# pvjosue/CWFA

Hardware: AMD Instinct MI355X
Metric: volumes/sec inverse-pass @512×512×96 fp32; NLL match vs ref (1/2/4/8 GPU) (higher is better)
Workload: dtype f32 (storage, accumulation, wavelets, couplings); convolution products on the bf16 matrix cores from an exact three-way bf16 split of both fp32 operands, six products per fp32 product: fp32-equivalent; plain-fp32-MFMA figure: fp32_mfma; 1 GPU; 512x512x96 volume, 4-scale CWFA (CAT blocks, 64 ch) + LRNN inverse, z=0, batch 1/GPU, random-init weights (BASELINE.json configs[2]); precision=split, parallelism=replicated x1 (independent volumes per GPU, no collective)

## Files before the change

cwfa_amd/_lib.py:

```python
import ctypes as C
import os

_HERE = os.path.dirname(os.path.abspath(__file__))
LIB_PATH = os.path.join(_HERE, "libcwfa_hip.so")

CLAMP = {"NONE": 0, "ATAN": 1, "TANH": 2, "SIGMOID": 3}
ACT = {None: 0, "none": 0, "elu": 1, "prelu": 2, "gelu": 3, "relu": 4}
CHAIN_MAX = 8

c_f32p = C.c_void_p
c_i64p = C.c_void_p
c_f64p = C.c_void_p


class AffineStage(C.Structure):
    _fields_ = [("s_raw", c_f32p), ("t", c_f32p), ("s_bs", C.c_int64), ("t_bs", C.c_int64), ("clamp_kind", C.c_int),
                ("clamp", C.c_float), ("pre_scale", C.c_float), ("t_neg_div_sqrt2", C.c_int), ("perm", c_i64p),
                ("perm_axis", C.c_int), ("gin", C.c_int)]


class Chain(C.Structure):
    _fields_ = [("n_stages", C.c_int), ("stage", AffineStage * CHAIN_MAX), ("src_c", C.c_void_p), ("src_h", C.c_void_p)]


# ... 45 lines not shown
    "cwfa_layernorm_apply_f32": (i, [p, p, p, p, f, p, i, i64, p]),
    "cwfa_attention_combine_f32": (i, [p, p, p, p, p, p, p, p, i, i, i64, p]),
    "cwfa_scale_channels_f32": (i, [p, p, p, i, i, i64, p]),
    "cwfa_axpby_f32": (i, [p, p, f, f, p, i64, p]),
    "cwfa_bn_running_update_f32": (i, [p, C.c_double, f, p, p, p, i, p]),
    "cwfa_bn_finish_f32": (i, [p, d, p, p, p, f, i, p, p, f, p, p, f, f, i, p, p, i, i, p]),
    "cwfa_chain_bwd_f32": (i, [p, p, C.POINTER(Chain), C.POINTER(ChainGrads), p, p, i, i, i, i, i64, i64, i64, f, f, i, p, p]),
    "cwfa_affine_bwd_f32": (i, [p, p, C.POINTER(AffineStage), i, i, i, i, i, i64, i64, p, p, p, p, p]),
    "cwfa_chain_inv_bwd_f32": (i, [p, p, C.POINTER(Chain), C.POINTER(ChainGrads), i, i, i, i, i64, i64, f, i, i, p, p, p, p]),
    "cwfa_conv2d_wgrad_workspace_bytes": (i64, [i, i, i, i, i, i]),
    "cwfa_conv2d_wgrad_f32": (i, [p, p, p, p, p, i, i, i, i, i, i, i64, i64, f, p]),
    "cwfa_elu_bwd_f32": (i, [p, p, p, p, i, i64, i64, i64, i64, i64, p]),
    "cwfa_conv3d_hidden_fwd_f32": (i, [p, p, p, p, i, i, i, i, i, p]),
    "cwfa_conv3d_hidden_bwd_f32": (i, [p, p, p, p, p, p, i, i, i, i, i, p]),
    "cwfa_conv3d_input_bwd_f32": (i, [p, p, p, i, i, i, i, i, p]),
    "cwfa_conv3d_wgrad_workspace_bytes": (i64, [i, i, i, i]),
    "cwfa_conv3d_wgrad_f32": (i, [p, p, p, p, p, i, i, i, i, i, i, i, f, p]),
    "cwfa_prelu_bwd_f32": (i, [p, p, p, p, p, i, i64, i64, i64, i64, p]),
    "cwfa_plane_affine_f32": (i, [p, p, p, i, p, p, i, i, i64, i64, i64, i64, p]),
    "cwfa_bn_bwd_stats_f32": (i, [p, p, p, p, i, i, i64, i64, i64, p]),
    "cwfa_bn_act_bwd_f32": (i, [p, p, p, i, p, p, p, p, p, i, i, i64, i64, i64, i64, p]),
    "cwfa_maxpool2_bwd_f32": (i, [p, p, p, p, i, i, i, i, p]),
    "cwfa_gelu_f32": (i, [p, p, p, i64, i, p]),
    "cwfa_layernorm_bwd_f32": (i, [p, p, p, p, p, p, p, p, p, i, i64, p]),
    "cwfa_attention_bwd_f32": (i, [p, p, p, p, p, p, p, p, p, i, i, i64, p]),
    "cwfa_split_workspace_bytes": (i64, [i, i, i64]),
    "cwfa_split_input_f32": (i, [p, p, i, i, i64, i64, p, p, i64, p, i64, p]),
    "cwfa_conv_split_packed_bytes": (i64, [i, i, i]),
    "cwfa_conv_split_pack_f32": (i, [p, p, i, i, i, i, p]),
    "cwfa_conv_split_f32": (i, [p, p, p, i, i, i, i, i, i, i64, C.POINTER(ConvOpts), p]),
    "cwfa_conv3x3_split_packed_bytes": (i64, [i, i]),
    "cwfa_conv3x3_split_pack_f32": (i, [p, p, i, i, p]),
    "cwfa_conv3x3_split_f32": (i, [p, p, p, i, i, i, i, i, i64, i64, C.POINTER(ConvOpts), p]),
    "cwfa_conv7x7_split_packed_bytes": (i64, [i, i]),
    "cwfa_conv7x7_split_pack_f32": (i, [p, p, i, i, p]),
    "cwfa_conv7x7_split_f32": (i, [p, p, p, i, i, i, i, i, i64, i64, C.POINTER(ConvOpts), p]),
    "cwfa_couple_rows": (i, [i, p]),
    "cwfa_conv3x3_split_couple_f32": (i, [p, p, p, i, i, i, i, i64, C.POINTER(Couple), p]),
    "cwfa_subnet_layer_split_packed_bytes": (i64, []),
    "cwfa_subnet_layer_split_pack_f32": (i, [p, p, p, p]),
    "cwfa_subnet_layer_split_f32": (i, [p, p, p, p, p, i, i, i, i64, i64, i, p]),
    "cwfa_subnet_layer_split_tape_f32": (i, [p, p, p, p, p, p, i, i, i, i64, i64, i64, p]),
    "cwfa_subnet_layer_first_packed_bytes": (i64, []),
    "cwfa_subnet_layer_first_pack_f32": (i, [p, p, p, i, p, p]),
    "cwfa_subnet_layer_first_f32": (i, [p, p, p, p, p, p, i, i, i, i, i64, i64, i64, i, p]),
    "cwfa_extract_views_f32": (i, [p, p, p, i, i, i, i, i, i, f, f, i64, p]),
}
del i, i64, f, d, p

_lib = None


class CwfaHipError(RuntimeError):
    pass


def lib():
    global _lib
    if _lib is None:
        if not os.path.exists(LIB_PATH):
            raise CwfaHipError(
                f"{LIB_PATH} not found: build the HIP extension first (python -m cwfa_amd.build, or "
                f"__graft_entry__.build()).  cwfa_amd has no CPU / PyTorch fallback.")
        import torch
        h = C.CDLL(LIB_PATH)
        for name, (res, args) in SIGNATURES.items():
# ... 14 lines not shown
```

cwfa_amd/csrc/conv_split3x3.hip:

```cpp
#include "conv_internal.h"

extern int g_cwfa_split_products;
extern int g_cwfa_split_xcd_map;
extern int g_cwfa_split_rows16;
extern int g_cwfa_split_operand;

namespace {

constexpr int TR = 8, TC = 32;

template <int KS, int RPW = 4>
struct XG {
    static constexpr int TRW = 2 * RPW, NT = 2 * RPW;
    static constexpr int PAD = KS / 2, XR = TRW + 2 * PAD, XC = TC + 2 * PAD, NTAP = KS * KS;
    static constexpr int EPK = XR * XC;
    static constexpr int KHB = KS == 7 ? 8512 : RPW == 8 ? 9792 : 5440;
    static constexpr int XPB = 2 * KHB;
    static constexpr int XB = 3 * XPB;
    static constexpr bool SPECIAL = KS == 3 && RPW == 4;
    static constexpr int NEK = SPECIAL ? 2 : 3;
    static_assert(EPK * 16 <= KHB && KHB % 256 == 64 && 2 * EPK <= 512 * NEK, "staging entry map");
    static_assert(!SPECIAL || (EPK > 256 && EPK <= 384), "3x3 staging entry map");
    static_assert(KS == 3 || RPW == 4, "7x7: 8-row tiles");
};
// ... 446 lines not shown
                                                            int nchunks, int nsteps, int64_t total, int ntap) {
    const int64_t i = (int64_t)blockIdx.x * blockDim.x + threadIdx.x;
    if (i >= total) return;
    const int col = (int)(i % CT), g = (int)((i / CT) % 4), s = (int)((i / (4 * CT)) % nsteps), ctile = (int)(i / ((int64_t)4 * CT * nsteps));
    const int u = 2 * s + (g >> 1), chunk = u / ntap, tap = u % ntap, co = ctile * CT + col;
    unsigned short pc[3][8];
#pragma unroll
    for (int j = 0; j < 8; ++j) {
        const int ci = chunk * 16 + (g & 1) * 8 + j;
        float v = 0.f;
        if (co < Cout && ci < Cin && chunk < nchunks) v = w[((int64_t)co * Cin + ci) * ntap + tap];
        __bf16 a1, a2, a3;
        if constexpr (F16) {
            cwfa_split3<false, true>(v, a1, a2, a3);
            a2 = a3 = __builtin_bit_cast(__bf16, (unsigned short)0);
        } else {
            cwfa_split3<true>(v, a1, a2, a3);
        }
        pc[0][j] = __builtin_bit_cast(unsigned short, a1);
        pc[1][j] = __builtin_bit_cast(unsigned short, a2);
        pc[2][j] = __builtin_bit_cast(unsigned short, a3);
    }
#pragma unroll
    for (int q = 0; q < 3; ++q) {
        uint4 v4;
        v4.x = pc[q][0] | ((unsigned)pc[q][1] << 16);
        v4.y = pc[q][2] | ((unsigned)pc[q][3] << 16);
        v4.z = pc[q][4] | ((unsigned)pc[q][5] << 16);
        v4.w = pc[q][6] | ((unsigned)pc[q][7] << 16);
        out[(((int64_t)ctile * nsteps + s) * 3 + q) * 4 * CT + g * CT + col] = v4;
    }
}

inline int mpw_of(int Cout) { return Cout > 128 ? 4 : Cout > 96 ? 2 : Cout > 64 ? 3 : Cout > 48 ? 1 : Cout > 32 ? 3 : Cout > 16 ? 2 : 1; }
inline int wm_of(int Cout) { return Cout > 96 ? 4 : Cout > 64 ? 2 : Cout > 48 ? 4 : 1; }
inline int ct_of(int Cout) { return 16 * mpw_of(Cout) * wm_of(Cout); }
inline int nsteps_of(int Cin, int ntap = 9) { return ntap * (((Cin + 15) / 16 + 1) / 2); }

template <int MPW, bool SIX, bool ADD, int ACT1, int KS = 3, int RPW = 4, int WM = 4, bool F16 = false>
int launch(const SParams& p, hipStream_t stream) {
    typedef Geo<MPW, KS, RPW, WM> G;
    constexpr int TRW = XG<KS, RPW>::TRW;
    auto kern = &conv3x3_split_kernel<MPW, SIX, ADD, ACT1, KS, RPW, WM, F16>;
    static bool attr_set = false;
    if (!attr_set) {
        hipError_t e = hipFuncSetAttribute(reinterpret_cast<const void*>(kern), hipFuncAttributeMaxDynamicSharedMemorySize, G::LDS);
        if (e != hipSuccess) {
            cwfa_set_error("cwfa_conv3x3_split_f32: hipFuncSetAttribute(%d bytes LDS): %s", G::LDS, hipGetErrorString(e));
            return CWFA_E_HIP;
        }
        attr_set = true;
    }
    const int tiles_y = (p.H + TRW - 1) / TRW, ctiles = (p.Cout + G::CT - 1) / G::CT;
    SParams q = p;
    q.ntiles = p.tiles_x * tiles_y;
    q.ctiles = ctiles;
    q.xcd_map = g_cwfa_split_xcd_map;
    if ((int64_t)q.ntiles * ctiles >= (1ll << 31)) {
        cwfa_set_error("cwfa_conv3x3_split_f32: grid too large");
        return CWFA_E_SHAPE;
    }
    hipLaunchKernelGGL(kern, dim3((unsigned)(q.ntiles * ctiles), 1, p.B), dim3(512), G::LDS, stream, q);
    CWFA_LAUNCH_CHECK("cwfa_conv3x3_split_f32");
    return CWFA_OK;
}

inline int split_op() { return g_cwfa_split_products != 1 ? 0 : g_cwfa_split_operand ? 2 : 1; }

template <int MPW, bool ADD, int ACT1, int KS = 3, int RPW = 4, int WM = 4>
int launch_op(int op, const SParams& p, hipStream_t st) {
    if (op == 0) return launch<MPW, true, ADD, ACT1, KS, RPW, WM>(p, st);
    if (op == 1) return launch<MPW, false, ADD, ACT1, KS, RPW, WM>(p, st);
    return launch<MPW, false, ADD, ACT1, KS, RPW, WM, true>(p, st);
}

template <int MPW>
int launch_epi(int op, const SParams& p, hipStream_t st) {
    const bool plain = !p.o.residual && p.o.act2 == CWFA_ACT_NONE;
    if (p.o.in_add) {
        if (plain && p.o.act == CWFA_ACT_PRELU) return launch_op<MPW, true, CWFA_ACT_PRELU>(op, p, st);
        return launch_op<MPW, true, EPI_RUNTIME>(op, p, st);
    }
    if (plain && p.o.act == CWFA_ACT_PRELU) return launch_op<MPW, false, CWFA_ACT_PRELU>(op, p, st);
    if (plain && p.o.act == CWFA_ACT_NONE) return launch_op<MPW, false, CWFA_ACT_NONE>(op, p, st);
    return launch_op<MPW, false, EPI_RUNTIME>(op, p, st);
}

}

static int couple_row_source(int n, int r) {
    int j, which;
    if (n <= 32) {
        const int wm = r >> 4, g = (r >> 2) & 3, q = r & 3;
        j = 8 * wm + 2 * g + (q & 1);
        which = q >> 1;
    } else {
        const int wm = r >> 5;
        which = (r >> 4) & 1;
        j = 16 * wm + (r & 15);
    }
    return j < n ? which * n + j : -1;
}

extern "C" int cwfa_couple_rows(int n, int* rows) {
    if (n <= 0 || n > 64) return -1;
    const int total = n <= 32 ? 64 : 128;
// ... 104 lines not shown
    CWFA_REQUIRE((int64_t)(Cin + 64) * H * W * 4 < (1ll << 31) && (int64_t)(Cout + 64 * mpw) * H * W * 4 < (1ll << 31) &&
                     (int64_t)(p.nsteps + 2) * 3 * 4 * 64 * mpw * 16 < (1ll << 31), CWFA_E_SHAPE,
                 "cwfa_conv3x3_split_f32: one sample's input / output / one cout tile's weights must stay below 2 GiB");
    CWFA_REQUIRE((int64_t)p.tiles_x * ((H + TR - 1) / TR) < (1ll << 31) && B <= 65535, CWFA_E_SHAPE, "cwfa_conv3x3_split_f32: grid too large");
    hipStream_t st = (hipStream_t)stream;
    const int op = split_op();
    const int wm = wm_of(Cout);
    if (wm != 4) {
        CWFA_REQUIRE(!p.o.in_scale && !p.o.in_add && !p.o.out_blocked8, CWFA_E_INVAL,
                     "cwfa_conv3x3_split_f32: banks with <= 48 or 65 .. 96 outputs take no load-side prologue and write NCHW");
        const bool plain = !p.o.residual && p.o.act2 == CWFA_ACT_NONE;
        const int epi = plain && p.o.act == CWFA_ACT_NONE ? 0 : plain && p.o.act == CWFA_ACT_PRELU ? 1 : 2;
#define CWFA_NARROW(M, W_)                                                                                                                   \
    do {                                                                                                                                     \
        if (epi == 0) return launch_op<M, false, CWFA_ACT_NONE, 3, 8, W_>(op, p, st);                                                    \
        if (epi == 1) return launch_op<M, false, CWFA_ACT_PRELU, 3, 8, W_>(op, p, st);                                                   \
        return launch_op<M, false, EPI_RUNTIME, 3, 8, W_>(op, p, st);                                                                    \
    } while (0)
        if (mpw == 3 && wm == 2) CWFA_NARROW(3, 2);
        if (mpw == 3) CWFA_NARROW(3, 1);
        if (mpw == 2) CWFA_NARROW(2, 1);
        CWFA_NARROW(1, 1);
#undef CWFA_NARROW
    }
    if (mpw == 4) return launch_epi<4>(op, p, st);
    if (mpw == 2) return launch_epi<2>(op, p, st);
    if (g_cwfa_split_rows16 && H > 8 && !p.o.in_scale && !p.o.in_add && !p.o.residual && p.o.act == CWFA_ACT_NONE && p.o.act2 == CWFA_ACT_NONE)
        return launch_op<2, false, CWFA_ACT_NONE, 3, 8, 2>(op, p, st);
    if (g_cwfa_split_rows16 && H > 8 && !p.o.in_scale && !p.o.in_add)
        return launch_op<2, false, EPI_RUNTIME, 3, 8, 2>(op, p, st);
    return launch_epi<1>(op, p, st);
}

extern "C" int64_t cwfa_conv7x7_split_packed_bytes(int Cout, int Cin) {
    if (Cout <= 0 || Cout > 64 || Cin <= 0) return -1;
    return (int64_t)nsteps_of(Cin, 49) * 3 * 4 * 64 * 16;
}

extern "C" int cwfa_conv7x7_split_pack_f32(const float* w, void* packed, int Cout, int Cin, void* stream) {
    CWFA_REQUIRE(w && packed, CWFA_E_INVAL, "cwfa_conv7x7_split_pack_f32: null pointer");
    CWFA_REQUIRE(Cout > 0 && Cout <= 64 && Cin > 0, CWFA_E_SHAPE, "cwfa_conv7x7_split_pack_f32: 1 <= Cout <= 64");
    CWFA_REQUIRE(cwfa_aligned16(packed), CWFA_E_ALIGN, "cwfa_conv7x7_split_pack_f32: packed image must be 16-byte aligned");
    const int nchunks = (Cin + 15) / 16, nsteps = nsteps_of(Cin, 49);
    const int64_t total = (int64_t)nsteps * 4 * 64;
    if (split_op() == 2)
        hipLaunchKernelGGL((split3x3_pack_kernel<64, true>), dim3((unsigned)((total + 255) / 256)), dim3(256), 0, (hipStream_t)stream, w,
                           reinterpret_cast<uint4*>(packed), Cout, Cin, nchunks, nsteps, total, 49);
    else
        hipLaunchKernelGGL(split3x3_pack_kernel<64>, dim3((unsigned)((total + 255) / 256)), dim3(256), 0, (hipStream_t)stream, w,
                           reinterpret_cast<uint4*>(packed), Cout, Cin, nchunks, nsteps, total, 49);
    CWFA_LAUNCH_CHECK("cwfa_conv7x7_split_pack_f32");
    return CWFA_OK;
}

extern "C" int cwfa_conv7x7_split_f32(const float* x, const void* w_packed, float* y, int B, int Cin, int H, int W, int Cout,
                                      int64_t x_bs, int64_t y_bs, const cwfa_conv_opts* opts, void* stream) {
    CWFA_REQUIRE(B >= 0 && Cin > 0 && Cout > 0 && Cout <= 64 && H >= 0 && W >= 0, CWFA_E_INVAL, "cwfa_conv7x7_split_f32: bad size (Cout <= 64)");
    if (B == 0 || H == 0 || W == 0) return CWFA_OK;
    CWFA_REQUIRE(x && w_packed && y, CWFA_E_INVAL, "cwfa_conv7x7_split_f32: null pointer");
    CWFA_REQUIRE(cwfa_aligned16(w_packed), CWFA_E_ALIGN, "cwfa_conv7x7_split_f32: packed weights must be 16-byte aligned");
    SParams p{};
    p.x = x; p.wp = w_packed; p.y = y;
    p.B = B; p.Cin = Cin; p.H = H; p.W = W; p.Cout = Cout; p.x_bs = x_bs; p.y_bs = y_bs;
    if (opts) p.o = *opts;
    CWFA_REQUIRE(!p.o.upshuffle2 && !p.o.in_cat && !p.o.in_scale && !p.o.in_add && !p.o.in_blocked8 && !p.o.out_blocked8 && !p.o.residual && !p.o.out_stats &&
                     p.o.act == CWFA_ACT_NONE && p.o.act2 == CWFA_ACT_NONE,
// ... 12 lines not shown
```

cwfa_amd/ops.py:

```python
import ctypes as C

import torch

from . import _lib
from ._lib import AffineStage, Chain, ConvOpts, check

__all__ = ["haar1d", "haar2d", "gather", "affine", "channel_affine", "chain_inv", "chain_fwd", "pack_conv_weight",
           "conv2d", "conv2d_wgrad", "elu_bwd", "set_precision", "gelu_add", "gelu_bwd", "layernorm_bwd", "attention_bwd", "plane_affine", "bn_bwd_stats", "bn_act_bwd", "maxpool2_bwd", "chain_bwd", "chain_inv_bwd", "prelu_bwd", "conv3d_1k1_backward", "pack_1x1_panel", "pack_split_layer_weight", "subnet_layer", "conv3d_1k1", "channel_stats", "bn_fold", "bn_running_update", "maxpool", "sample_stats", "layernorm_apply",
           "attention_combine", "scale_channels", "axpby", "stage"]


def _stream():
    return C.c_void_p(torch.cuda.current_stream().cuda_stream)


def _p(t):
    return None if t is None else C.c_void_p(t.data_ptr())


def _dev(t, name="tensor"):
    if not torch.is_tensor(t):
        raise TypeError(f"{name}: expected a torch.Tensor, got {type(t)}")
    if not t.is_cuda:
        raise RuntimeError(f"{name}: cwfa_amd runs on MI355X only -- got a {t.device} tensor (no CPU fallback exists)")
# ... 279 lines not shown
    loss = torch.zeros(1, dtype=torch.float64, device=xhat.device)
    if want_low_grad and loss_kind != 0:
        raise ValueError("chain_inv_bwd: dL/dlow is formed from an upstream gradient (loss_kind 0)")
    gz = torch.empty((B, Cc, H, W), dtype=torch.float32, device=xhat.device) if want_latent_grad else None
    glow = torch.empty((B, Cc, H, W), dtype=torch.float32, device=xhat.device) if want_low_grad else None
    check(L.cwfa_chain_inv_bwd_f32(_p(xhat), _p(gt), C.byref(ch), C.byref(gr), B, Cc, H, W, xbs, gbs, float(gscale), int(loss_kind),
                                   int(bool(accumulate)), _p(loss), _p(gz), _p(glow), _stream()), "chain_inv_bwd")
    if want_latent_grad or want_low_grad:
        return loss, gz, glow
    return loss


def chain_bwd(z, stages, grads, final_perm=None, gscale=0.0, ldscale=0.0, gz=None, want_input_grad=False, accumulate=False, gld=None):
    L = _lib.lib()
    z, zbs = planes(z, "z")
    B, Cc, H, W = z.shape
    ch, keep = _chain(stages)
    gr = _chain_grads(grads, (B, Cc, H, W))
    gzbs = 0
    if gz is not None:
        gz, gzbs = planes(gz, "gz")
    gv0 = torch.empty((B, Cc, H, W), dtype=torch.float32, device=z.device) if want_input_grad else None
    if gld is not None:
        gld = _dev(gld, "gld").contiguous()
        if gld.numel() != B:
            raise ValueError("chain_bwd: gld must hold one value per sample")
    check(L.cwfa_chain_bwd_f32(_p(z), _p(gz), C.byref(ch), C.byref(gr), _p(_idx(final_perm)), _p(gv0), B, Cc, H, W, zbs, gzbs,
                               Cc * H * W, float(gscale), float(ldscale), int(bool(accumulate)), _p(gld), _stream()), "chain_bwd")
    return gv0


class PackedConv:
    __slots__ = ("packed", "cout", "cin", "ks", "transposed", "version", "src_ptr", "split", "epoch", "version1", "src_ptr1", "cat_c1",
                 "cat_from", "short")

    def __init__(self, packed, cout, cin, ks, transposed, version, src_ptr, split=False):
        self.packed, self.cout, self.cin, self.ks = packed, cout, cin, ks
        self.transposed, self.version, self.src_ptr = transposed, version, src_ptr
        self.split = split
        self.epoch = _pack_epoch


def pack_conv_weight(w, transposed=False, direct=False):
    L = _lib.lib()
    w = _dev(w, "weight").detach().contiguous()
    if transposed:
        cin, co, kh, kw = w.shape
        if (kh, kw) != (2, 2):
            raise ValueError("only 2x2 stride-2 transposed convolutions are supported")
        cout, ks = 4 * co, 1
    else:
        cout, cin, ks, kw = w.shape
        if ks != kw:
            raise ValueError("square kernels only")
    if direct:
        pass
    elif _split_bf16 and ks == 1 and cout >= 128:
        packed = torch.empty(L.cwfa_conv_split_packed_bytes(cout, cin, ks), dtype=torch.uint8, device=w.device)
        check(L.cwfa_conv_split_pack_f32(_p(w), _p(packed), cout, cin, ks, int(transposed), _stream()), "conv_split_pack")
        return PackedConv(packed, cout, cin, ks, transposed, w._version, w.data_ptr(), split=True)
    narrow_max = 32 if single_product() else SPLIT_3X3_NARROW_MAX
    if not direct and _split_bf16 >= 2 and ks == 3 and cout >= SPLIT_3X3_MIN_COUT and (cout > 32 or (cout <= narrow_max and cin >= 29)):
        packed = torch.empty(L.cwfa_conv3x3_split_packed_bytes(cout, cin), dtype=torch.uint8, device=w.device)
        check(L.cwfa_conv3x3_split_pack_f32(_p(w), _p(packed), cout, cin, _stream()), "conv3x3_split_pack")
        return PackedConv(packed, cout, cin, ks, transposed, w._version, w.data_ptr(), split=True)
    if not direct and SPLIT_7X7 and _split_bf16 >= 2 and ks == 7 and cout <= 64 and cin >= 32:
        packed = torch.empty(L.cwfa_conv7x7_split_packed_bytes(cout, cin), dtype=torch.uint8, device=w.device)
        check(L.cwfa_conv7x7_split_pack_f32(_p(w), _p(packed), cout, cin, _stream()), "conv7x7_split_pack")
        return PackedConv(packed, cout, cin, ks, transposed, w._version, w.data_ptr(), split=True)
    n = L.cwfa_conv2d_packed_floats(cout, cin, ks)
    if n <= 0:
        raise ValueError(f"unsupported filter bank {tuple(w.shape)}")
    packed = torch.empty(n, dtype=torch.float32, device=w.device)
    check(L.cwfa_conv2d_pack_f32(_p(w), _p(packed), cout, cin, ks, int(transposed), _stream()), "conv2d_pack")
    return PackedConv(packed, cout, cin, ks, transposed, w._version, w.data_ptr())


def pack_conv_weight_cat(w, c1):
    w = _dev(w, "weight").detach()
    cout, cin, ks, kw = w.shape
    if ks != 1 or kw != 1 or cout > 64 or not (0 < c1 < cin):
        raise ValueError(f"pack_conv_weight_cat: a 1x1 bank with <= 64 outputs and 0 < c1 < Cin is needed, got {tuple(w.shape)}, c1 = {c1}")
    start = (c1 + 15) // 16 * 16
    wz = torch.zeros((cout, start + cin - c1, 1, 1), dtype=torch.float32, device=w.device)
    wz[:, :c1] = w[:, :c1]
    wz[:, start:] = w[:, c1:]
    pc = pack_conv_weight(wz)
    pc.version, pc.src_ptr = w._version, w.data_ptr()
    pc.cat_c1, pc.cat_from = c1, start
# ... 81 lines not shown
            raise ValueError("conv2d: out_stats must be a float64 [2*Cout] tensor on the HIP device")
        o.out_stats = out_stats.data_ptr()
    rec = conv_event_sink
    if rec is not None:
        key = (pc.ks, Cin, pc.cout, H, W, B, "%s|%s|%s|%s|%s" % ("pro" if (in_scale is not None or in_add is not None) else "",
                                                                 act or "", "res" if residual is not None else "", act2 or "",
                                                                 ("up" if up else "") + ("+split" if pc.split else "")),
               in_add is not None)
        if rec.want(key):
            e0, e1 = torch.cuda.Event(enable_timing=True), torch.cuda.Event(enable_timing=True)
            e0.record()
    if pc.split and pc.ks == 7:
        if act or act2 or residual is not None or in_scale is not None or in_add is not None:
            raise ValueError("conv2d: the split-bf16 7x7 kernel has a bias-only epilogue and no load-side prologue")
        check(L.cwfa_conv7x7_split_f32(_p(x), _p(pc.packed), _p(out), B, Cin, H, W, pc.cout, xbs, ybs, C.byref(o), _stream()),
              "conv7x7_split")
    elif pc.split and pc.ks == 3:
        if split3x3_narrow(pc.cout) and (in_scale is not None or in_add is not None):
            if (H * W) % 4 == 0:
                x = plane_affine(x, in_scale, in_shift, add=in_add)
            else:
                if in_scale is not None:
                    if in_scale.numel() == Cin:
                        x = channel_affine(x, in_scale.reshape(-1), in_shift.reshape(-1))
                    else:
                        x = torch.cat([channel_affine(x[i:i + 1], in_scale.reshape(B, Cin)[i].contiguous(), in_shift.reshape(B, Cin)[i].contiguous())
                                       for i in range(B)], 0)
                if in_add is not None:
                    x = axpby(x.contiguous(), 1.0, in_add, 1.0)
            x, xbs = planes(x, "x")
            o.in_scale = o.in_shift = o.in_add = None
        check(L.cwfa_conv3x3_split_f32(_p(x), _p(pc.packed), _p(out), B, Cin, H, W, pc.cout, xbs, ybs, C.byref(o),
                                       _stream()), "conv3x3_split")
    elif pc.split:
        ws = torch.empty(L.cwfa_split_workspace_bytes(B, Cin, H * W), dtype=torch.uint8, device=x.device)
        per_sample = in_scale is not None and in_scale.numel() == B * Cin and B > 1
        check(L.cwfa_split_input_f32(_p(x), _p(ws), B, Cin, H * W, xbs, _p(in_scale), _p(in_shift), Cin if per_sample else 0,
                                     _p(in_add), in_add.stride(0) if in_add is not None else 0, _stream()), "split_input")
        o.in_scale = o.in_shift = o.in_add = None
        check(L.cwfa_conv_split_f32(_p(ws), _p(pc.packed), _p(out), B, Cin, H, W, pc.cout, pc.ks, ybs, C.byref(o), _stream()),
              "conv_split")
    else:
        check(L.cwfa_conv2d_f32(_p(x), _p(pc.packed), _p(out), B, Cin, H, W, pc.cout, pc.ks, xbs, ybs, C.byref(o),
                                _stream()), "conv2d")
    if rec is not None and rec.want(key):
        e1.record()
        rec.add(key, e0, e1)
    return out


def pack_couple_weight(w, bias):
    L = _lib.lib()
    w = _dev(w, "weight").detach()
    n2, cin, ks, kw = w.shape
    if ks != 3 or kw != 3 or n2 % 2 or n2 // 2 > 64:
        raise ValueError(f"pack_couple_weight: a [2n,Cin,3,3] bank with n <= 64 is needed, got {tuple(w.shape)}")
    n = n2 // 2
    total = L.cwfa_couple_rows(n, None)
    rows_c = (C.c_int * total)()
    L.cwfa_couple_rows(n, rows_c)
    rows = torch.tensor(list(rows_c), dtype=torch.int64, device=w.device)
    live = (rows >= 0)
    wr = torch.zeros((total, cin, 3, 3), dtype=torch.float32, device=w.device)
    wr[live] = w[rows[live]]
    br = torch.zeros(total, dtype=torch.float32, device=w.device)
    if bias is not None:
# ... 689 lines not shown
```

include/cwfa_hip.h:

```cpp
#ifndef CWFA_HIP_H
#define CWFA_HIP_H

#include <stdint.h>

#ifdef __cplusplus
extern "C" {
#endif

#define CWFA_VERSION 100

enum {
    CWFA_OK = 0,
    CWFA_E_INVAL = -1,
    CWFA_E_SHAPE = -2,
    CWFA_E_ALIGN = -3,
    CWFA_E_HIP = -4
};

enum { CWFA_CLAMP_NONE = 0, CWFA_CLAMP_ATAN = 1, CWFA_CLAMP_TANH = 2, CWFA_CLAMP_SIGMOID = 3 };

enum { CWFA_ACT_NONE = 0, CWFA_ACT_ELU = 1, CWFA_ACT_PRELU = 2, CWFA_ACT_GELU = 3, CWFA_ACT_RELU = 4 };

int cwfa_version(void);
const char* cwfa_last_error(void);
// ... 100 lines not shown


int cwfa_channel_stats_f32(const float* x, double* stats, int B, int C, int64_t HW, int64_t x_bs, void* stream);
int cwfa_bn_fold_f32(const double* stats, double count, const float* running_mean, const float* running_var,
                     const float* weight, const float* bias, float eps, const float* mask_bc, int B, float* scale,
                     float* shift, int C, void* stream);
int cwfa_bn_finish_f32(double* stats, double count, float* running_mean, float* running_var, long long* num_batches_tracked,
                       float momentum, int update_running, const float* weight, const float* bias, float eps, const float* mask_bc,
                       const float* mask_u, float drop_p, float keep_scale, int B, float* scale, float* shift, int C, int zero_stats,
                       void* stream);
int cwfa_bn_running_update_f32(const double* stats, double count, float momentum, float* running_mean, float* running_var,
                               long long* num_batches_tracked, int C, void* stream);
int cwfa_maxpool_f32(const float* x, float* y, float* full, const float* scale, const float* shift, int B, int C,
                     int H, int W, int Ho, int Wo, void* stream);
int cwfa_sample_stats_f32(const float* x, double* stats, int B, int64_t CHW, void* stream);
int cwfa_layernorm_apply_f32(const float* x, const double* stats, const float* w, const float* b, float eps,
                             float* y, int B, int64_t CHW, void* stream);
int cwfa_attention_combine_f32(const float* mean, const float* w1, const float* b1, const float* w2, const float* b2,
                               const float* m, const float* x, float* out, int B, int C, int64_t HW, void* stream);
int cwfa_scale_channels_f32(const float* x, const float* scale_bc, float* y, int B, int C, int64_t HW, void* stream);
int cwfa_axpby_f32(const float* x, const float* z, float a, float b, float* y, int64_t n, void* stream);

int64_t cwfa_split_workspace_bytes(int B, int Cin, int64_t HW);
int cwfa_split_input_f32(const float* x, void* ws, int B, int Cin, int64_t HW, int64_t x_bs, const float* in_scale,
                         const float* in_shift, int64_t in_affine_bs, const float* in_add, int64_t in_add_bs, void* stream);
int64_t cwfa_conv_split_packed_bytes(int Cout, int Cin, int ks);
int cwfa_conv_split_pack_f32(const float* w, void* packed, int Cout, int Cin, int ks, int transposed, void* stream);
int64_t cwfa_conv3x3_split_packed_bytes(int Cout, int Cin);
int cwfa_conv3x3_split_pack_f32(const float* w, void* packed, int Cout, int Cin, void* stream);
int cwfa_conv3x3_split_f32(const float* x, const void* w_packed, float* y, int B, int Cin, int H, int W, int Cout,
                           int64_t x_bs, int64_t y_bs, const cwfa_conv_opts* opts, void* stream);
int cwfa_conv_split_f32(const void* ws, const void* w_packed, float* y, int B, int Cin, int H, int W, int Cout, int ks, int64_t y_bs,
                           const cwfa_conv_opts* opts, void* stream);
int64_t cwfa_conv7x7_split_packed_bytes(int Cout, int Cin);
int cwfa_conv7x7_split_pack_f32(const float* w, void* packed, int Cout, int Cin, void* stream);
int cwfa_conv7x7_split_f32(const float* x, const void* w_packed, float* y, int B, int Cin, int H, int W, int Cout,
                           int64_t x_bs, int64_t y_bs, const cwfa_conv_opts* opts, void* stream);

typedef struct {
    const float* x;
    float* y;
    int64_t x_bs, y_bs;
    int n;
    int clamp_kind;
    float clamp, pre_scale;
    int rev;
    double* logdet;
    int in_blocked8;
} cwfa_couple;
int cwfa_couple_rows(int n, int* rows);
int cwfa_conv3x3_split_couple_f32(const float* x, const void* w_packed, const float* bias_rows, int B, int Cin, int H, int W,
                                  int64_t x_bs, const cwfa_couple* cp, void* stream);

int64_t cwfa_subnet_layer_split_packed_bytes(void);
int cwfa_subnet_layer_split_pack_f32(const float* w3, const float* w1, void* packed, void* stream);
int cwfa_subnet_layer_split_f32(const float* x, const void* packed, const float* b3, const float* b1, float* y, int B, int H,
                                int W, int64_t x_bs, int64_t y_bs, int layout, void* stream);
int64_t cwfa_subnet_layer_first_packed_bytes(void);
int cwfa_subnet_layer_first_pack_f32(const float* w3c, const float* w1, const float* w0c, int short_form, void* packed, void* stream);
int cwfa_subnet_layer_first_f32(const float* u, const float* x, const void* packed, const float* b3, const float* b1, float* y, int B,
                                int u_ch, int H, int W, int64_t u_bs, int64_t x_bs, int64_t y_bs, int layout, void* stream);
int cwfa_subnet_layer_split_tape_f32(const float* x, const void* packed, const float* b3, const float* b1, float* y, float* hid, int B,
                                     int H, int W, int64_t x_bs, int64_t y_bs, int64_t hid_bs, void* stream);

int cwfa_extract_views_f32(const float* image, const int* coords_yx, float* views, int B, int Hs, int Ws, int nviews, int sh,
                           int sw, float mean, float stdv, int64_t image_bs, void* stream);
// ... 59 lines not shown
```

Baseline: 53.11 volumes/s.

## Add fused 1x1 split-bf16 conv kernel for wide outputs

Adds a dedicated 1x1 convolution kernel for Cout>=128 in the six-product split-bf16 path. It splits the fp32 input into three bf16 parts inside the kernel, applying any input affine and add there, instead of writing a separate split workspace first. Weights stream into double-buffered LDS via buffer-to-LDS DMA while the matrix-core products run, and there is an optional fused upshuffle epilogue. This removes the extra split pass and its workspace memory traffic, at the cost of a large LDS footprint (one block per CU) and a new hand-scheduled pipeline.

```diff
diff --git a/cwfa_amd/_lib.py b/cwfa_amd/_lib.py
--- a/cwfa_amd/_lib.py
+++ b/cwfa_amd/_lib.py
@@ -101,6 +101,9 @@
     "cwfa_conv3x3_split_packed_bytes": (i64, [i, i]),
     "cwfa_conv3x3_split_pack_f32": (i, [p, p, i, i, p]),
     "cwfa_conv3x3_split_f32": (i, [p, p, p, i, i, i, i, i, i64, i64, C.POINTER(ConvOpts), p]),
+    "cwfa_conv1x1_split_packed_bytes": (i64, [i, i]),
+    "cwfa_conv1x1_split_pack_f32": (i, [p, p, i, i, p]),
+    "cwfa_conv1x1_split_f32": (i, [p, p, p, i, i, i, i, i, i64, i64, C.POINTER(ConvOpts), p]),
     "cwfa_conv7x7_split_packed_bytes": (i64, [i, i]),
     "cwfa_conv7x7_split_pack_f32": (i, [p, p, i, i, p]),
     "cwfa_conv7x7_split_f32": (i, [p, p, p, i, i, i, i, i, i64, i64, C.POINTER(ConvOpts), p]),
diff --git a/cwfa_amd/csrc/conv_split3x3.hip b/cwfa_amd/csrc/conv_split3x3.hip
--- a/cwfa_amd/csrc/conv_split3x3.hip
+++ b/cwfa_amd/csrc/conv_split3x3.hip
@@ -502,6 +502,223 @@
     }
 }
 
+constexpr int G1_KP = 128 * 16 + 64;
+constexpr int G1_XPB = 4 * G1_KP;
+constexpr int G1_XB = 3 * G1_XPB;
+template <int MPW>
+struct Geo1 {
+    static constexpr int CT = 64 * MPW, WSL = 3 * 4 * CT * 16;
+    static constexpr int LDS = 2 * G1_XB + 2 * WSL;
+    static_assert(LDS <= 160 * 1024, "LDS budget");
+};
+
+__device__ __forceinline__ void store_b64(float a, float b, __amdgpu_buffer_rsrc_t rsrc, unsigned voffset, int soffset) {
+    typedef unsigned u32x2 __attribute__((ext_vector_type(2)));
+    __builtin_amdgcn_raw_buffer_store_b64(u32x2{__builtin_bit_cast(unsigned, a), __builtin_bit_cast(unsigned, b)}, rsrc, voffset, soffset, 0);
+    asm volatile("s_nop 1");
+    __builtin_amdgcn_sched_barrier(0);
+}
+
+template <int MPW, bool ADD, bool UP>
+__global__ __launch_bounds__(512, 1) void conv1x1_split16_kernel(SParams p) {
+    constexpr int CT = 64 * MPW, WSL = Geo1<MPW>::WSL, NT = 4, RW = 2, TRW = 4;
+    constexpr int OFF_W = 2 * G1_XB;
+    extern __shared__ __attribute__((aligned(16))) char lds[];
+    const int tid = threadIdx.x, lane = tid & 63, c16 = lane & 15, g = lane >> 4;
+    const int wave = __builtin_amdgcn_readfirstlane(tid >> 6);
+    const int wm = wave & 3, wn = wave >> 2;
+    const int HW = p.H * p.W;
+    const int plane = HW * 4;
+    constexpr unsigned OOB = 0x80000000u;
+    const int b = blockIdx.z;
+    int sp, ct;
+    if (p.xcd_map && (p.ntiles & 7) == 0) {
+        const int xcd = blockIdx.x & 7, slot = blockIdx.x >> 3;
+        sp = xcd * (p.ntiles >> 3) + slot / p.ctiles;
+        ct = slot % p.ctiles;
+    } else {
+        sp = blockIdx.x / p.ctiles;
+        ct = blockIdx.x % p.ctiles;
+    }
+    const int row0 = (sp / p.tiles_x) * TRW, col0 = (sp % p.tiles_x) * TC;
+
+    const int kg = wave >> 1, px = tid & 127;
+    const int gr = row0 + (px >> 5), gc = col0 + (px & 31);
+    const unsigned fo = gr < p.H && gc < p.W ? (unsigned)((gr * p.W + gc) * 4) : OOB;
+    const int xbytes = p.Cin * plane;
+    const auto rx = CWFA_RSRC(p.x + (int64_t)b * p.x_bs, xbytes);
+    const auto ra = CWFA_RSRC(ADD ? p.o.in_add + (int64_t)b * p.o.in_add_bs : p.x, ADD ? xbytes : 0);
+    const bool has_aff = p.o.in_scale != nullptr;
+    typedef const float __attribute__((address_space(4))) cfloat;
+    cfloat* sc = has_aff ? (cfloat*)(p.o.in_scale + (int64_t)b * p.o.in_affine_bs) : nullptr;
+    cfloat* sh = has_aff ? (cfloat*)(p.o.in_shift + (int64_t)b * p.o.in_affine_bs) : nullptr;
+    float xv[8], av[8];
+    auto load_entry = [&](int step) {
+        const int ch0 = step * 32 + kg * 8;
+#pragma unroll
+        for (int j = 0; j < 8; ++j) xv[j] = __builtin_bit_cast(float, __builtin_amdgcn_raw_buffer_load_b32(rx, fo, (ch0 + j) * plane, 0));
+        if constexpr (ADD) {
+#pragma unroll
+            for (int j = 0; j < 8; ++j) av[j] = __builtin_bit_cast(float, __builtin_amdgcn_raw_buffer_load_b32(ra, fo, (ch0 + j) * plane, 0));
+        }
+    };
+    auto store_entry = [&](int step, int buf) {
+        const int ch0 = step * 32 + kg * 8;
+        float scv[8], shv[8];
+        if (has_aff) {
+#pragma unroll
+            for (int j = 0; j < 8; ++j) {
+                const int ch = ch0 + j < p.Cin ? ch0 + j : p.Cin - 1;
+                scv[j] = sc[ch];
+                shv[j] = sh[ch];
+            }
+        }
+        bf16x8 pc[3];
+#pragma unroll
+        for (int j = 0; j < 8; ++j) {
+            float v = xv[j];
+            if (has_aff) v = v * scv[j] + shv[j];
+            if constexpr (ADD) v += av[j];
+            __bf16 a1, a2, a3;
+            cwfa_split3<true>(v, a1, a2, a3);
+            pc[0][j] = a1; pc[1][j] = a2; pc[2][j] = a3;
+        }
+        char* dst = lds + buf * G1_XB + kg * G1_KP + px * 16;
+#pragma unroll
+        for (int q = 0; q < 3; ++q) *reinterpret_cast<bf16x8*>(dst + q * G1_XPB) = pc[q];
+    };
+
+    constexpr int NPC = WSL / 1024;
+    const char* wbase = reinterpret_cast<const char*>(p.wp) + (int64_t)ct * p.nsteps * WSL;
+    const auto rw = CWFA_RSRC(wbase, p.nsteps * WSL);
+    auto dma_w = [&](int slice, int slot) {
+        cwfa_static_for<(NPC + 7) / 8>([&](auto ic_) {
+            constexpr int i = decltype(ic_)::value;
+            const int piece = i * 8 + wave;
+            if (piece < NPC) {
+                char* dst = lds + OFF_W + slot * WSL + piece * 1024;
+                __builtin_amdgcn_raw_ptr_buffer_load_lds(rw, (lds_ptr)dst, 16, (unsigned)(lane * 16), slice * WSL + piece * 1024, 0, 0);
+            }
+        });
+    };
+
+    const int alane = OFF_W + (g * CT + wm * MPW * 16 + c16) * 16;
+    const int blane = g * G1_KP + (wn * RW * TC + c16) * 16;
+
+    f32x4 acc[MPW][NT];
+#pragma unroll
+    for (int mt = 0; mt < MPW; ++mt)
+#pragma unroll
+        for (int nt = 0; nt < NT; ++nt) acc[mt][nt] = f32x4{0.f, 0.f, 0.f, 0.f};
+    bf16x8 A[MPW][3], Bq[2][3];
+    auto read_b = [&](int set, int bbase, int nt) {
+#pragma unroll
+        for (int q = 0; q < 3; ++q) Bq[set][q] = *reinterpret_cast<const bf16x8*>(lds + bbase + q * G1_XPB + nt * 256);
+    };
+    auto mfma6 = [&](f32x4& c, const bf16x8 (&a)[3], const bf16x8 (&bb)[3]) {
+        CWFA_MFMA(a[2], bb[0], c);
+        CWFA_MFMA(a[1], bb[1], c);
+        CWFA_MFMA(a[0], bb[2], c);
+        CWFA_MFMA(a[1], bb[0], c);
+        CWFA_MFMA(a[0], bb[1], c);
+        CWFA_MFMA(a[0], bb[0], c);
+    };
+
+    load_entry(0);
+    dma_w(0, 0);
+    store_entry(0, 0);
+    load_entry(1);
+    asm volatile("s_waitcnt vmcnt(0)\n\ts_waitcnt lgkmcnt(0)" ::: "memory");
+    __builtin_amdgcn_s_barrier();
+
+    for (int step = 0; step < p.nsteps; ++step) {
+        const int buf = step & 1;
+        const int abase = alane + buf * WSL;
+        const int bbase = blane + buf * G1_XB;
+        auto read_a = [&](int mt) {
+#pragma unroll
+            for (int q = 0; q < 3; ++q) A[mt][q] = *reinterpret_cast<const bf16x8*>(lds + abase + (q * 4 * CT + mt * 16) * 16);
+        };
+        read_a(0);
+        read_b(0, bbase, 0);
+#pragma unroll
+        for (int mt = 1; mt < MPW; ++mt) read_a(mt);
+        CWFA_FENCE();
+        if (step + 1 < p.nsteps) store_entry(step + 1, buf ^ 1);
+        CWFA_FENCE();
+        if (step + 2 < p.nsteps) load_entry(step + 2);
+        CWFA_FENCE();
+#pragma unroll
+        for (int nt = 0; nt < NT; ++nt) {
+            if (nt + 1 < NT) read_b((nt + 1) & 1, bbase, nt + 1);
+            CWFA_FENCE();
+#pragma unroll
+            for (int mt = 0; mt < MPW; ++mt) {
+                mfma6(acc[mt][nt], A[mt], Bq[nt & 1]);
+                CWFA_FENCE();
+            }
+            if (nt == 1) {
+                if (step + 1 < p.nsteps) dma_w(step + 1, buf ^ 1);
+                CWFA_FENCE();
+            }
+        }
+        asm volatile("s_waitcnt vmcnt(0)\n\ts_waitcnt lgkmcnt(0)" ::: "memory");
+        __builtin_amdgcn_s_barrier();
+    }
+
+    const int cwave = ct * CT + wm * MPW * 16;
+    const auto ry = CWFA_RSRC(p.y + (int64_t)b * p.y_bs, p.Cout * plane);
+    if constexpr (UP) {
+        const int W2 = 2 * p.W;
+        const auto rb = CWFA_RSRC(p.o.bias ? p.o.bias : p.y, p.o.bias ? (p.Cout >> 2) * 4 : 0);
+#pragma unroll
+        for (int mt = 0; mt < MPW; ++mt) {
+            const int cw = (cwave + mt * 16) >> 2;
+            const float bias = __builtin_bit_cast(float, __builtin_amdgcn_raw_buffer_load_b32(rb, (unsigned)(4 * g), cw * 4, 0));
+#pragma unroll
+            for (int nt = 0; nt < NT; ++nt) {
+                const int row = row0 + wn * RW + (nt >> 1), col = col0 + 16 * (nt & 1) + c16;
+                const unsigned po = row < p.H && col < p.W ? (unsigned)((2 * row * W2 + 2 * col) * 4) + (unsigned)g * (unsigned)(4 * plane) : OOB;
+                store_b64(acc[mt][nt][0] + bias, acc[mt][nt][1] + bias, ry, po, cw * 4 * plane);
+                store_b64(acc[mt][nt][2] + bias, acc[mt][nt][3] + bias, ry, po + (po == OOB ? 0u : (unsigned)(W2 * 4)), cw * 4 * plane);
+            }
+        }
+        return;
+    }
+    const auto rr = CWFA_RSRC(p.o.residual ? p.o.residual + (int64_t)b * p.o.res_bs : p.y, p.o.residual ? p.Cout * plane : 0);
+    const auto rb = CWFA_RSRC(p.o.bias ? p.o.bias : p.y, p.o.bias ? p.Cout * 4 : 0);
+    const float alpha = p.o.prelu_alpha ? *p.o.prelu_alpha : 0.f;
+    const unsigned glane = (unsigned)(4 * g) * (unsigned)plane;
+#pragma unroll
+    for (int mt = 0; mt < MPW; ++mt) {
+        float bias[4];
+#pragma unroll
+        for (int r = 0; r < 4; ++r)
+            bias[r] = __builtin_bit_cast(float, __builtin_amdgcn_raw_buffer_load_b32(rb, (unsigned)(16 * g), (cwave + mt * 16 + r) * 4, 0));
+#pragma unroll
+        for (int nt = 0; nt < NT; ++nt) {
+            const int row = row0 + wn * RW + (nt >> 1), col = col0 + 16 * (nt & 1) + c16;
+            const unsigned po = row < p.H && col < p.W ? (unsigned)((row * p.W + col) * 4) + glane : OOB;
+            float rv[4] = {0.f, 0.f, 0.f, 0.f};
+            if (p.o.residual) {
+#pragma unroll
+                for (int r = 0; r < 4; ++r)
+                    rv[r] = __builtin_bit_cast(float, __builtin_amdgcn_raw_buffer_load_b32(rr, po, (cwave + mt * 16 + r) * plane, 0));
+            }
+#pragma unroll
+            for (int r = 0; r < 4; ++r) {
+                float v = cwfa_act(acc[mt][nt][r] + bias[r], p.o.act, alpha);
+                v += rv[r];
+                v = cwfa_act(v, p.o.act2, alpha);
+                __builtin_amdgcn_raw_buffer_store_b32(__builtin_bit_cast(unsigned, v), ry, po, (cwave + mt * 16 + r) * plane, 0);
+            }
+            CWFA_FENCE();
+        }
+    }
+}
+
+inline int ct1_of(int Cout) { return Cout > 128 ? 256 : 128; }
+
 inline int mpw_of(int Cout) { return Cout > 128 ? 4 : Cout > 96 ? 2 : Cout > 64 ? 3 : Cout > 48 ? 1 : Cout > 32 ? 3 : Cout > 16 ? 2 : 1; }
 inline int wm_of(int Cout) { return Cout > 96 ? 4 : Cout > 64 ? 2 : Cout > 48 ? 4 : 1; }
 inline int ct_of(int Cout) { return 16 * mpw_of(Cout) * wm_of(Cout); }
@@ -542,6 +759,40 @@
     if (op == 0) return launch<MPW, true, ADD, ACT1, KS, RPW, WM>(p, st);
     if (op == 1) return launch<MPW, false, ADD, ACT1, KS, RPW, WM>(p, st);
     return launch<MPW, false, ADD, ACT1, KS, RPW, WM, true>(p, st);
+}
+
+template <int MPW, bool ADD, bool UP>
+int launch1(const SParams& p, hipStream_t stream) {
+    typedef Geo1<MPW> G;
+    auto kern = &conv1x1_split16_kernel<MPW, ADD, UP>;
+    static bool attr_set = false;
+    if (!attr_set) {
+        hipError_t e = hipFuncSetAttribute(reinterpret_cast<const void*>(kern), hipFuncAttributeMaxDynamicSharedMemorySize, G::LDS);
+        if (e != hipSuccess) {
+            cwfa_set_error("cwfa_conv1x1_split_f32: hipFuncSetAttribute(%d bytes LDS): %s", G::LDS, hipGetErrorString(e));
+            return CWFA_E_HIP;
+        }
+        attr_set = true;
+    }
+    const int tiles_y = (p.H + 3) / 4, ctiles = (p.Cout + G::CT - 1) / G::CT;
+    SParams q = p;
+    q.ntiles = p.tiles_x * tiles_y;
+    q.ctiles = ctiles;
+    q.xcd_map = g_cwfa_split_xcd_map;
+    if ((int64_t)q.ntiles * ctiles >= (1ll << 31)) {
+        cwfa_set_error("cwfa_conv1x1_split_f32: grid too large");
+        return CWFA_E_SHAPE;
+    }
+    hipLaunchKernelGGL(kern, dim3((unsigned)(q.ntiles * ctiles), 1, p.B), dim3(512), G::LDS, stream, q);
+    CWFA_LAUNCH_CHECK("cwfa_conv1x1_split_f32");
+    return CWFA_OK;
+}
+
+template <int MPW>
+int launch1_epi(const SParams& p, hipStream_t st) {
+    const bool up = p.o.upshuffle2 != 0;
+    if (p.o.in_add) return up ? launch1<MPW, true, true>(p, st) : launch1<MPW, true, false>(p, st);
+    return up ? launch1<MPW, false, true>(p, st) : launch1<MPW, false, false>(p, st);
 }
 
 template <int MPW>
@@ -712,6 +963,60 @@
     return launch_epi<1>(op, p, st);
 }
 
+extern "C" int64_t cwfa_conv1x1_split_packed_bytes(int Cout, int Cin) {
+    if (Cout <= 0 || Cin <= 0) return -1;
+    const int ct = ct1_of(Cout);
+    return (int64_t)((Cout + ct - 1) / ct) * nsteps_of(Cin, 1) * 3 * 4 * ct * 16;
+}
+
+extern "C" int cwfa_conv1x1_split_pack_f32(const float* w, void* packed, int Cout, int Cin, void* stream) {
+    CWFA_REQUIRE(w && packed, CWFA_E_INVAL, "cwfa_conv1x1_split_pack_f32: null pointer");
+    CWFA_REQUIRE(Cout > 0 && Cin > 0, CWFA_E_SHAPE, "cwfa_conv1x1_split_pack_f32: bad shape");
+    CWFA_REQUIRE(cwfa_aligned16(packed), CWFA_E_ALIGN, "cwfa_conv1x1_split_pack_f32: packed image must be 16-byte aligned");
+    CWFA_REQUIRE(split_op() == 0, CWFA_E_INVAL, "cwfa_conv1x1_split_pack_f32: split_products = 6 only (one product: cwfa_conv_split_pack_f32)");
+    const int ct = ct1_of(Cout), nchunks = (Cin + 15) / 16, nsteps = nsteps_of(Cin, 1);
+    const int64_t total = (int64_t)((Cout + ct - 1) / ct) * nsteps * 4 * ct;
+    const dim3 grid((unsigned)((total + 255) / 256));
+    uint4* out = reinterpret_cast<uint4*>(packed);
+    if (ct == 256) hipLaunchKernelGGL(split3x3_pack_kernel<256>, grid, dim3(256), 0, (hipStream_t)stream, w, out, Cout, Cin, nchunks, nsteps, total, 1);
+    else hipLaunchKernelGGL(split3x3_pack_kernel<128>, grid, dim3(256), 0, (hipStream_t)stream, w, out, Cout, Cin, nchunks, nsteps, total, 1);
+    CWFA_LAUNCH_CHECK("cwfa_conv1x1_split_pack_f32");
+    return CWFA_OK;
+}
+
+extern "C" int cwfa_conv1x1_split_f32(const float* x, const void* w_packed, float* y, int B, int Cin, int H, int W, int Cout,
+                                      int64_t x_bs, int64_t y_bs, const cwfa_conv_opts* opts, void* stream) {
+    CWFA_REQUIRE(B >= 0 && Cin > 0 && Cout > 0 && H >= 0 && W >= 0, CWFA_E_INVAL, "cwfa_conv1x1_split_f32: bad size");
+    if (B == 0 || H == 0 || W == 0) return CWFA_OK;
+    CWFA_REQUIRE(x && w_packed && y, CWFA_E_INVAL, "cwfa_conv1x1_split_f32: null pointer");
+    CWFA_REQUIRE(cwfa_aligned16(w_packed), CWFA_E_ALIGN, "cwfa_conv1x1_split_f32: packed weights must be 16-byte aligned");
+    CWFA_REQUIRE(split_op() == 0, CWFA_E_INVAL, "cwfa_conv1x1_split_f32: split_products = 6 only (one product: cwfa_conv_split_f32)");
+    SParams p{};
+    p.x = x; p.wp = w_packed; p.y = y;
+    p.B = B; p.Cin = Cin; p.H = H; p.W = W; p.Cout = Cout; p.x_bs = x_bs; p.y_bs = y_bs;
+    if (opts) p.o = *opts;
+    CWFA_REQUIRE(!p.o.in_cat && !p.o.in_blocked8 && !p.o.out_blocked8 && !p.o.out_stats && !p.o.prelu_per_channel, CWFA_E_INVAL,
+                 "cwfa_conv1x1_split_f32: NCHW maps, one source, no statistics, one PReLU slope");
+    CWFA_REQUIRE(!p.o.upshuffle2 || (Cout % 4 == 0 && !p.o.residual && p.o.act == CWFA_ACT_NONE && p.o.act2 == CWFA_ACT_NONE), CWFA_E_INVAL,
+                 "cwfa_conv1x1_split_f32: upshuffle2 needs Cout = 4*Co and a bias-only epilogue");
+    CWFA_REQUIRE(!(p.o.in_scale && !p.o.in_shift), CWFA_E_INVAL, "cwfa_conv1x1_split_f32: in_scale without in_shift");
+    CWFA_REQUIRE(p.o.act >= 0 && p.o.act <= CWFA_ACT_RELU && p.o.act2 >= 0 && p.o.act2 <= CWFA_ACT_RELU, CWFA_E_INVAL,
+                 "cwfa_conv1x1_split_f32: bad activation");
+    CWFA_REQUIRE(!((p.o.act == CWFA_ACT_PRELU || p.o.act2 == CWFA_ACT_PRELU) && !p.o.prelu_alpha), CWFA_E_INVAL,
+                 "cwfa_conv1x1_split_f32: PReLU without prelu_alpha");
+    p.nchunks = (Cin + 15) / 16;
+    p.nsteps = nsteps_of(Cin, 1);
+    p.nrun = p.nsteps;
+    p.tiles_x = (W + TC - 1) / TC;
+    const int ct = ct1_of(Cout);
+    CWFA_REQUIRE((int64_t)(Cin + 64) * H * W * 4 < (1ll << 31) && (int64_t)(Cout + 256) * H * W * 4 < (1ll << 31) &&
+                     (int64_t)(p.nsteps + 2) * 3 * 4 * ct * 16 < (1ll << 31), CWFA_E_SHAPE,
+                 "cwfa_conv1x1_split_f32: one sample's input / output / one cout tile's weights must stay below 2 GiB");
+    CWFA_REQUIRE((int64_t)p.tiles_x * ((H + 3) / 4) < (1ll << 31) && B <= 65535, CWFA_E_SHAPE, "cwfa_conv1x1_split_f32: grid too large");
+    hipStream_t st = (hipStream_t)stream;
+    return ct == 256 ? launch1_epi<4>(p, st) : launch1_epi<2>(p, st);
+}
+
 extern "C" int64_t cwfa_conv7x7_split_packed_bytes(int Cout, int Cin) {
     if (Cout <= 0 || Cout > 64 || Cin <= 0) return -1;
     return (int64_t)nsteps_of(Cin, 49) * 3 * 4 * 64 * 16;
diff --git a/cwfa_amd/ops.py b/cwfa_amd/ops.py
--- a/cwfa_amd/ops.py
+++ b/cwfa_amd/ops.py
@@ -335,13 +335,14 @@
 
 class PackedConv:
     __slots__ = ("packed", "cout", "cin", "ks", "transposed", "version", "src_ptr", "split", "epoch", "version1", "src_ptr1", "cat_c1",
-                 "cat_from", "short")
+                 "cat_from", "short", "gemm16")
 
     def __init__(self, packed, cout, cin, ks, transposed, version, src_ptr, split=False):
         self.packed, self.cout, self.cin, self.ks = packed, cout, cin, ks
         self.transposed, self.version, self.src_ptr = transposed, version, src_ptr
         self.split = split
         self.epoch = _pack_epoch
+        self.gemm16 = False
 
 
 def pack_conv_weight(w, transposed=False, direct=False):
@@ -358,6 +359,13 @@
             raise ValueError("square kernels only")
     if direct:
         pass
+    elif _split_bf16 and ks == 1 and cout >= 128 and not single_product():
+        w2 = w.permute(1, 2, 3, 0).reshape(cout, cin).contiguous() if transposed else w.reshape(cout, cin)
+        packed = torch.empty(L.cwfa_conv1x1_split_packed_bytes(cout, cin), dtype=torch.uint8, device=w.device)
+        check(L.cwfa_conv1x1_split_pack_f32(_p(w2), _p(packed), cout, cin, _stream()), "conv1x1_split_pack")
+        pc = PackedConv(packed, cout, cin, ks, transposed, w._version, w.data_ptr(), split=True)
+        pc.gemm16 = True
+        return pc
     elif _split_bf16 and ks == 1 and cout >= 128:
         packed = torch.empty(L.cwfa_conv_split_packed_bytes(cout, cin, ks), dtype=torch.uint8, device=w.device)
         check(L.cwfa_conv_split_pack_f32(_p(w), _p(packed), cout, cin, ks, int(transposed), _stream()), "conv_split_pack")
@@ -505,6 +513,9 @@
             o.in_scale = o.in_shift = o.in_add = None
         check(L.cwfa_conv3x3_split_f32(_p(x), _p(pc.packed), _p(out), B, Cin, H, W, pc.cout, xbs, ybs, C.byref(o),
                                        _stream()), "conv3x3_split")
+    elif pc.split and pc.gemm16:
+        check(L.cwfa_conv1x1_split_f32(_p(x), _p(pc.packed), _p(out), B, Cin, H, W, pc.cout, xbs, ybs, C.byref(o), _stream()),
+              "conv1x1_split")
     elif pc.split:
         ws = torch.empty(L.cwfa_split_workspace_bytes(B, Cin, H * W), dtype=torch.uint8, device=x.device)
         per_sample = in_scale is not None and in_scale.numel() == B * Cin and B > 1
diff --git a/include/cwfa_hip.h b/include/cwfa_hip.h
--- a/include/cwfa_hip.h
+++ b/include/cwfa_hip.h
@@ -156,6 +156,10 @@
                            int64_t x_bs, int64_t y_bs, const cwfa_conv_opts* opts, void* stream);
 int cwfa_conv_split_f32(const void* ws, const void* w_packed, float* y, int B, int Cin, int H, int W, int Cout, int ks, int64_t y_bs,
                            const cwfa_conv_opts* opts, void* stream);
+int64_t cwfa_conv1x1_split_packed_bytes(int Cout, int Cin);
+int cwfa_conv1x1_split_pack_f32(const float* w, void* packed, int Cout, int Cin, void* stream);
+int cwfa_conv1x1_split_f32(const float* x, const void* w_packed, float* y, int B, int Cin, int H, int W, int Cout,
+                           int64_t x_bs, int64_t y_bs, const cwfa_conv_opts* opts, void* stream);
 int64_t cwfa_conv7x7_split_packed_bytes(int Cout, int Cin);
 int cwfa_conv7x7_split_pack_f32(const float* w, void* packed, int Cout, int Cin, void* stream);
 int cwfa_conv7x7_split_f32(const float* x, const void* w_packed, float* y, int B, int Cin, int H, int W, int Cout,
```

Result: no change. 53.27 volumes/s, median of 6 (+0.3%).
